# zerenluo123/legged_gym

Measured on AMD Instinct MI355X. Metric: env-steps/sec (whole node), Go1 rough-terrain 4096 envs/GPU at 1/2/4/8 GPUs, higher is better.
Workload: dtype fp32; 1 GPU; C3 go1_rough: Go1 trimesh curriculum terrain + 187-point height scan, actuator-net history+MLP, PPO 24 steps x 4096 envs/GPU, 5 epochs x 4 minibatches; envs_per_gpu=4096, global_envs=4096, parallelism=dp1

## Files before the change

legged_gym_amd/csrc/lgx_api.hip:

```cpp
#include <stdio.h>
#include <string.h>

#include <new>
#include <string>
#include <vector>

#include "lgx_internal.h"

static thread_local std::string g_err;

static int fail(int code, const char* msg) {
  g_err = msg;
  return code;
}
static int hip_check(hipError_t e, const char* what) {
  if (e == hipSuccess) return 0;
  char buf[256];
  snprintf(buf, sizeof buf, "%s: %s", what, hipGetErrorString(e));
  g_err = buf;
  return LGX_EHIP;
}
int lgx_fail(int code, const char* msg) { return fail(code, msg); }
int lgx_hip_status(const char* what) { return hip_check(hipGetLastError(), what); }
static int launch_check(int rc, const char* what) {
  if (rc == 0) return 0;
  if (rc == -1) return fail(LGX_EINVAL, what);
  return hip_check(hipGetLastError(), what);
}

struct lgx_sim {
  int device;
  bool dense;
  int pp;
  int act_mode;
  int32_t num_points;
  lgx_env_params params;
  lgx_buffers bufs;
  lgx_dev_model* d_model;
  lgx_env_params* d_params;
  const float* draws;
  float* extras_snapshot;
  lgx_priv_args priv;
  lgx_hist_args hist;
  lgx_act_rand_args arand;
  hipStream_t aux;
  hipEvent_t aux_in, aux_done;
  bool aux_pending;
  int32_t n_term_rows;
  int32_t profiling;
  int64_t prof_calls;
  std::vector<hipEvent_t> ev[3];
  std::vector<hipEvent_t> pool;
};

static hipEvent_t take_event(lgx_sim* s) {
  if (!s->pool.empty()) { hipEvent_t e = s->pool.back(); s->pool.pop_back(); return e; }
  hipEvent_t e = nullptr;
  if (hipEventCreateWithFlags(&e, hipEventDisableSystemFence) != hipSuccess) return nullptr;
  return e;
}
thread_local lgx_timing_slot lgx_timing;

static void arm(lgx_sim* s, int cls, bool sample) {
  lgx_timing = lgx_timing_slot{};
  if (!sample) return;
  hipEvent_t e0 = take_event(s), e1 = take_event(s);
// ... 80 lines not shown
  lgx_dev_model dm;
  memset(&dm, 0, sizeof dm);
  dm.m = *model;
  dm.m.leg_dof = leg_dof;
  int rr = 0;
  for (int i = 0; i < (dense ? 0 : model->num_points); ++i) {
    int d = model->point_dyn[i];
    int rep = model->point_report[i];
    if (d < 0 || d >= LGX_NUM_DYN) return fail(LGX_EINVAL, "lgx_sim_create: bad point_dyn");
    int lane;
    if (d == 0) {
      if (rep != 0) return fail(LGX_EINVAL, "lgx_sim_create: base points must report on body 0");
      lane = rr++ & 3;
    } else {
      lane = (d - 1) / 3;
      if (rep < 1 + 4 * lane || rep > 4 + 4 * lane) return fail(LGX_EINVAL, "lgx_sim_create: leg point reports on a foreign body");
    }
    if (dm.lane_npts[lane] >= LGX_MAX_LANE_PTS) return fail(LGX_EINVAL, "lgx_sim_create: too many contact points per leg");
    dm.lane_pts[lane][dm.lane_npts[lane]++] = i;
  }
  for (int l = 0; l < 4; ++l) dm.max_lane_npts = dm.lane_npts[l] > dm.max_lane_npts ? dm.lane_npts[l] : dm.max_lane_npts;
  dm.joint_rot_eye = 1;
  for (int j = 0; j < LGX_NUM_DOF; ++j)
    for (int i = 0; i < 9; ++i)
      if (model->joint_rot[j][i] != (i % 4 == 0 ? 1.f : 0.f)) dm.joint_rot_eye = 0;

  int rc = hip_check(hipSetDevice(device), "hipSetDevice");
  if (rc) return rc;
  lgx_sim* s = new (std::nothrow) lgx_sim();
  if (!s) return fail(LGX_ENOMEM, "lgx_sim_create: out of host memory");
  s->device = device;
  s->dense = dense;
  s->pp = lgx_physics_pp(params->num_envs);
  const char* am = getenv("LGX_ACT_OVERLAP");
  s->act_mode = am && *am ? atoi(am) : 2;
  if (s->act_mode < 0 || s->act_mode > 2 || (am && *am && (am[0] < '0' || am[0] > '2' || am[1]))) {
    delete s;
    return fail(LGX_EINVAL, "lgx_sim_create: LGX_ACT_OVERLAP must be 0, 1 or 2");
  }
  s->num_points = model->num_points;
  s->params = *params;
  s->bufs = *bufs;
  s->draws = nullptr;
  s->extras_snapshot = nullptr;
  s->priv = lgx_priv_args{};
  s->hist = lgx_hist_args{};
  s->arand = lgx_act_rand_args{};
  s->aux = nullptr;
  s->aux_in = s->aux_done = nullptr;
  s->aux_pending = false;
  s->profiling = 0;
  s->prof_calls = 0;
  s->n_term_rows = params->num_terms + (params->termination_slot >= 0 ? 1 : 0);
  if ((rc = hip_check(hipMalloc(&s->d_model, sizeof(lgx_dev_model)), "hipMalloc(model)"))) { delete s; return rc; }
  if ((rc = hip_check(hipMalloc(&s->d_params, sizeof(lgx_env_params)), "hipMalloc(params)"))) {
    (void)hipFree(s->d_model); delete s; return rc;
  }
  rc = hip_check(hipMemcpy(s->d_model, &dm, sizeof dm, hipMemcpyHostToDevice), "hipMemcpy(model)");
  if (!rc) rc = hip_check(hipMemcpy(s->d_params, params, sizeof *params, hipMemcpyHostToDevice), "hipMemcpy(params)");
  if (!rc) {
    const int64_t blocks = (params->num_envs + LGX_ENV_BLOCK - 1) / LGX_ENV_BLOCK;
    rc = hip_check(hipMemset(bufs->scratch + blocks * LGX_PARTIAL_STRIDE, 0, sizeof(unsigned int)), "hipMemset(ticket)");
  }
  if (rc) { (void)hipFree(s->d_model); (void)hipFree(s->d_params); delete s; return rc; }
  *out = s;
  return 0;
// ... 179 lines not shown
  if (ctrl == LGX_CTRL_T && (d->kp_scale || d->kd_scale))
    return fail(LGX_EINVAL, "lgx_bind_actuator_rand: LGX_CTRL_T has no gains to scale");
  const size_t bytes = sizeof(float) * (size_t)s->params.num_envs * LGX_NUM_DOF;
  float* prev = s->arand.prev;
  if (!prev) {
    if (int rc = hip_check(hipMalloc(&prev, bytes), "lgx_bind_actuator_rand: hipMalloc(prev)")) return rc;
  }
  s->arand = lgx_act_rand_args{d->kp_scale, d->kd_scale, d->lag, prev};
  if (int rc = hip_check(hipDeviceSynchronize(), "lgx_bind_actuator_rand: hipDeviceSynchronize")) return rc;
  if (int rc = hip_check(hipMemset(prev, 0, bytes), "lgx_bind_actuator_rand: hipMemset(prev)")) return rc;
  return hip_check(hipDeviceSynchronize(), "lgx_bind_actuator_rand: hipDeviceSynchronize");
}

int lgx_rebind_extras(lgx_sim* s, float* snapshot) {
  if (!s) return fail(LGX_EINVAL, "lgx_rebind_extras: null sim");
  s->extras_snapshot = snapshot;
  return 0;
}

static int join_aux(lgx_sim* s, hipStream_t st) {
  if (!s->aux_pending) return 0;
  return hip_check(hipStreamWaitEvent(st, s->aux_done, 0), "hipStreamWaitEvent(aux)");
}


int lgx_sync_aux(lgx_sim* s, void* stream) {
  if (!s) return fail(LGX_EINVAL, "lgx_sync_aux: null sim");
  return join_aux(s, (hipStream_t)stream);
}

static int physics(lgx_sim* s, int32_t nsub, int32_t from_actions, const float* actions, hipStream_t st, int32_t frozen) {
  if (s->arand.prev)
    return lgx_launch_physics_rand(s->d_model, s->d_params, s->bufs, s->params.num_envs, nsub, from_actions, actions,
                                   st, frozen, s->pp, s->arand);
  return s->dense ? lgx_launch_physics_dense(s->d_model, s->d_params, s->bufs, s->params.num_envs, nsub, from_actions,
                                             actions, st, frozen, s->num_points)
                  : lgx_launch_physics(s->d_model, s->d_params, s->bufs, s->params.num_envs, nsub, from_actions, actions,
                                       st, frozen, s->pp);
}

int lgx_simulate(lgx_sim* s, int32_t n, void* stream) {
  if (!s || n < 0) return fail(LGX_EINVAL, "lgx_simulate: bad arguments");
  if (n == 0) return 0;
  if (int rc = join_aux(s, (hipStream_t)stream)) return rc;
  return launch_check(physics(s, n, 0, nullptr, (hipStream_t)stream, 0), "lgx_simulate: physics launch");
}

int lgx_drive_inputs(lgx_sim* s, const float* actions, void* stream) {
  if (!s) return fail(LGX_EINVAL, "lgx_drive_inputs: null sim");
  if (int rc = join_aux(s, (hipStream_t)stream)) return rc;
  return launch_check(physics(s, s->params.decimation, 1, actions, (hipStream_t)stream, 1), "lgx_drive_inputs: launch");
}

int lgx_ground_contact(lgx_sim* s, const float* points, int32_t n, float* out, void* stream) {
  if (!s || n < 0 || (n > 0 && (!points || !out))) return fail(LGX_EINVAL, "lgx_ground_contact: bad arguments");
  return launch_check(lgx_launch_ground_contact(s->d_params, s->bufs, points, n, out, (hipStream_t)stream),
                      "lgx_ground_contact: launch");
}

int lgx_post_physics(lgx_sim* s, int64_t step, void* stream) {
  if (!s) return fail(LGX_EINVAL, "lgx_post_physics: null sim");
  return launch_check(lgx_launch_post_physics(s->d_params, s->bufs, s->params.num_envs, s->params.num_obs, s->n_term_rows,
                                              s->params.measure_heights, step, s->draws, s->extras_snapshot, s->priv,
                                              s->hist, (hipStream_t)stream),
                      "lgx_post_physics: launch");
}

static int post_physics_fused(lgx_sim* s, int64_t step, hipStream_t st, bool sample);

int lgx_step(lgx_sim* s, int64_t step, void* stream) { return lgx_step_from(s, nullptr, step, stream); }

// ... 200 lines not shown
```

legged_gym_amd/csrc/lgx_device.h:

```cpp
#pragma once
#include <hip/hip_runtime.h>
#include <stdint.h>

#include "../../include/lgx.h"

#define LGX_DEV __device__ __forceinline__

#ifdef LGX_PHASE_CLOCK
#include <stdio.h>
#define LGX_CLK_DECL(n) LGX_CLK_START uint64_t lgx_clk_acc[n] = {}; uint64_t lgx_clk_t = clock64();
#define LGX_CLK(i) do { const uint64_t _t = clock64(); lgx_clk_acc[i] += _t - lgx_clk_t; lgx_clk_t = _t; } while (0)
#ifdef LGX_PHASE_CLOCK_ALL
#define LGX_CLK_WHO (threadIdx.x == 0)
#else
#define LGX_CLK_WHO (blockIdx.x == 0 && threadIdx.x == 0)
#endif
#ifdef LGX_PHASE_CLOCK_BUF
#define LGX_CLK_MAXB 4096
static __device__ unsigned long long lgx_clk_buf[LGX_CLK_MAXB][14];
#define LGX_CLK_START const unsigned long long lgx_clk_t0 = __builtin_amdgcn_s_memrealtime();
#define LGX_CLK_PRINT(name, n)                                                                        \
  if (threadIdx.x == 0 && blockIdx.x < LGX_CLK_MAXB) {                                                \
    lgx_clk_buf[blockIdx.x][0] = lgx_clk_t0;                                                          \
    lgx_clk_buf[blockIdx.x][1] = __builtin_amdgcn_s_memrealtime();                                    \
    for (int _i = 0; _i < n && _i < 12; ++_i) lgx_clk_buf[blockIdx.x][2 + _i] = lgx_clk_acc[_i];      \
  }
#else
#define LGX_CLK_START
#define LGX_CLK_PRINT(name, n)                                                                        \
  if (LGX_CLK_WHO) {      \
    unsigned long long _v[12] = {};                                                                   \
    for (int _i = 0; _i < n && _i < 12; ++_i) _v[_i] = lgx_clk_acc[_i];                               \
    printf("%s cycles: b=%d 0=%llu 1=%llu 2=%llu 3=%llu 4=%llu 5=%llu 6=%llu 7=%llu 8=%llu 9=%llu "   \
           "10=%llu 11=%llu\n", name, (int)blockIdx.x, _v[0], _v[1], _v[2], _v[3], _v[4], _v[5], _v[6],  \
           _v[7], _v[8], _v[9], _v[10], _v[11]);                                                       \
  }
#endif
#else
#define LGX_CLK_DECL(n)
#define LGX_CLK(i) do { } while (0)
#define LGX_CLK_PRINT(name, n)
#endif

LGX_DEV void lgx_uniform4(uint64_t seed, int32_t env, int32_t slot4, int64_t step, uint32_t tag, float out[4]) {
  uint32_t c0 = (uint32_t)env, c1 = (uint32_t)slot4, c2 = (uint32_t)step;
  uint32_t c3 = tag ^ ((uint32_t)((uint64_t)step >> 32) << 8);
  uint32_t k0 = (uint32_t)seed, k1 = (uint32_t)(seed >> 32);
#pragma unroll
  for (int r = 0; r < 10; ++r) {
    uint32_t lo0 = 0xD2511F53u * c0, hi0 = __umulhi(0xD2511F53u, c0);
    uint32_t lo1 = 0xCD9E8D57u * c2, hi1 = __umulhi(0xCD9E8D57u, c2);
    uint32_t n0 = hi1 ^ c1 ^ k0, n2 = hi0 ^ c3 ^ k1;
    c0 = n0; c1 = lo1; c2 = n2; c3 = lo0;
    k0 += 0x9E3779B9u; k1 += 0xBB67AE85u;
  }
  const float s = 1.0f / 16777216.0f;
  out[0] = (float)(c0 >> 8) * s; out[1] = (float)(c1 >> 8) * s;
  out[2] = (float)(c2 >> 8) * s; out[3] = (float)(c3 >> 8) * s;
// ... 127 lines not shown
```

legged_gym_amd/csrc/lgx_internal.h:

```cpp
#pragma once
#include <hip/hip_ext.h>
#include <hip/hip_runtime.h>

#include "../../include/lgx.h"

#define LGX_MAX_LANE_PTS 24

struct lgx_dev_model {
  lgx_model m;
  int32_t lane_npts[4];
  int32_t max_lane_npts;
  int32_t joint_rot_eye;
  int32_t lane_pts[4][LGX_MAX_LANE_PTS];
  int32_t pad_tail[(4 - (sizeof(lgx_model) / 4 + 6 + 4 * LGX_MAX_LANE_PTS) % 4) % 4];
};

int lgx_launch_ground_contact(const lgx_env_params* dp, const lgx_buffers& b, const float* q, int32_t n, float* o,
                              hipStream_t stream);
int lgx_physics_pp(int32_t n_envs);
int lgx_launch_physics(const lgx_dev_model* dm, const lgx_env_params* dp, const lgx_buffers& b, int32_t n_envs,
                       int32_t nsub, int32_t from_actions, const float* act_src, hipStream_t stream, int32_t frozen,
                       int pp);
struct lgx_act_rand_args {
  const float* kp_scale;
  const float* kd_scale;
  const int32_t* lag;
  float* prev;
};
int lgx_launch_physics_rand(const lgx_dev_model* dm, const lgx_env_params* dp, const lgx_buffers& b, int32_t n_envs,
                            int32_t nsub, int32_t from_actions, const float* act_src, hipStream_t stream,
                            int32_t frozen, int pp, const lgx_act_rand_args& ar);
int lgx_launch_physics_dense(const lgx_dev_model* dm, const lgx_env_params* dp, const lgx_buffers& b, int32_t n_envs,
                             int32_t nsub, int32_t from_actions, const float* act_src, hipStream_t stream,
                             int32_t frozen, int32_t num_points);
struct lgx_priv_args {
  float* buf;
  int32_t width, num_terms;
  uint32_t ids;
  uint32_t pad;
  uint64_t offs_lo, offs_hi;
  float cf_scale, tq_scale;
  __host__ __device__ int id(int t) const { return (int)((ids >> (4 * t)) & 15u); }
  __host__ __device__ int off(int t) const { return (int)(((t < 4 ? offs_lo : offs_hi) >> (16 * (t & 3))) & 0xffffu); }
  void set(int t, int id_, int off_) {
    ids |= (uint32_t)id_ << (4 * t);
    (t < 4 ? offs_lo : offs_hi) |= (uint64_t)off_ << (16 * (t & 3));
  }
};
static_assert(LGX_PRIV_MAX_TERMS <= 8 && LGX_PRIV_COUNT <= 16 && LGX_MAX_PRIV_OBS < 65536, "lgx_priv_args packing");
struct lgx_hist_args {
  float* row;
  const float* prev;
  int32_t* age;
  int32_t frames, frame_width, width;
};
int lgx_launch_post_physics(const lgx_env_params* dp, const lgx_buffers& b, int32_t n_envs, int32_t num_obs,
                            int32_t n_term_rows, int32_t measure_heights, int64_t step, const float* draws,
                            float* extras_snapshot, const lgx_priv_args& pv, const lgx_hist_args& hv,
                            hipStream_t stream);
int lgx_launch_post_physics_act(const lgx_env_params* dp, const lgx_buffers& b, int32_t n_envs, int64_t step,
                                const float* draws, float* extras_snapshot, const float* act_in, float* act_out,
                                int64_t act_rows, const float* act_w, const float* act_scale,
                                const lgx_priv_args& pv, const lgx_hist_args& hv, hipStream_t stream);
int lgx_launch_post_physics_hist(const lgx_env_params* dp, const lgx_buffers& b, int32_t n_envs, int64_t step,
// ... 84 lines not shown
```

legged_gym_amd/csrc/lgx_physics.hip:

```cpp
#include <stdlib.h>

#include "lgx_device.h"
#include "lgx_internal.h"

namespace {

struct sv { f3 a, l; };
LGX_DEV sv sv0() { return sv{mk3(0, 0, 0), mk3(0, 0, 0)}; }
LGX_DEV sv add(sv x, sv y) { return sv{x.a + y.a, x.l + y.l}; }
LGX_DEV sv scale(float s, sv x) { return sv{s * x.a, s * x.l}; }
LGX_DEV float dot(sv x, sv y) { return dot(x.a, y.a) + dot(x.l, y.l); }
LGX_DEV sv crm(sv V, sv s) { return sv{cross(V.a, s.a), cross(V.a, s.l) + cross(V.l, s.a)}; }
LGX_DEV sv crf(sv V, sv f) { return sv{cross(V.a, f.a) + cross(V.l, f.l), cross(V.a, f.l)}; }

struct SI { float m; f3 h; float I[6]; };
LGX_DEV SI si_add(const SI& x, const SI& y) {
  SI r; r.m = x.m + y.m; r.h = x.h + y.h;
#pragma unroll
  for (int i = 0; i < 6; ++i) r.I[i] = x.I[i] + y.I[i];
  return r;
}
LGX_DEV sv si_mul(const SI& s, sv v) {
  f3 Ia = mk3(s.I[0] * v.a.x + s.I[3] * v.a.y + s.I[4] * v.a.z, s.I[3] * v.a.x + s.I[1] * v.a.y + s.I[5] * v.a.z,
              s.I[4] * v.a.x + s.I[5] * v.a.y + s.I[2] * v.a.z);
  return sv{Ia + cross(s.h, v.l), cross(v.a, s.h) + s.m * v.l};
}
LGX_DEV SI body_si(const lgx_model* __restrict__ M, int b, float scale, const m33& R, f3 o) {
  const float* in = M->body_inertia[b];
  m33 Ib = {{in[0], in[3], in[4], in[3], in[1], in[5], in[4], in[5], in[2]}};
  m33 T = mul(R, Ib);
  float Iw[6];
  Iw[0] = T.a[0] * R.a[0] + T.a[1] * R.a[1] + T.a[2] * R.a[2];
  Iw[1] = T.a[3] * R.a[3] + T.a[4] * R.a[4] + T.a[5] * R.a[5];
// ... 514 lines not shown
}

LGX_DEV void wave_lds_sync() {
  __builtin_amdgcn_fence(__ATOMIC_RELEASE, "wavefront");
  __builtin_amdgcn_wave_barrier();
  __builtin_amdgcn_fence(__ATOMIC_ACQUIRE, "wavefront");
}

}

#define MAX_LANE_PTS LGX_MAX_LANE_PTS
#ifndef LGX_PHYS_WAVES_PER_SIMD
#define LGX_PHYS_WAVES_PER_SIMD 1
#endif
#define HIST_STRIDE 31

template <int PP>
LGX_DEV float psum(float v) {
  if (PP == 4) return row_quads_sum(v);
  if (PP >= 2) v += lane_xor4(v);
  if (PP >= 4) v += lane_xor8(v);
  if (PP >= 8) v += __shfl_xor(v, 16);
  return v;
}

#define PHYS_KP(k, j) (RAND ? arow[k] : M->kp[j])
#define PHYS_KD(k, j) (RAND ? arow[3 + (k)] : M->kd[j])
#define PHYS_PG(k, j) (RAND ? arow[k] : P->p_gains[j])
#define PHYS_DG(k, j) (RAND ? arow[3 + (k)] : P->d_gains[j])
#define PHYS_AE(k) (RAND ? ae_lag[k] : act[k])
LGX_DEV lgx_act_rand_args act_rand_of() { return lgx_act_rand_args{nullptr, nullptr, nullptr, nullptr}; }
LGX_DEV lgx_act_rand_args act_rand_of(const lgx_act_rand_args& a) { return a; }

template <int PP, typename... AR>
__global__ void __launch_bounds__(64 * PP, LGX_PHYS_WAVES_PER_SIMD)
lgx_physics_kernel(const lgx_dev_model* __restrict__ DMg, const lgx_env_params* __restrict__ P, lgx_buffers B,
                   int32_t nsub, int32_t from_actions, const float* __restrict__ act_src, int32_t frozen, AR... ar) {
  static_assert(sizeof...(AR) <= 1, "at most the actuator tables");
  constexpr bool RAND = sizeof...(AR) == 1;
  constexpr int PHYS_BLOCK = 64 * PP;
  constexpr int LPE = 4 * PP;
  constexpr int SLOTS = (MAX_LANE_PTS + PP - 1) / PP;
  constexpr int ENVS = 16;
  __shared__ lgx_dev_model smodel;
  __shared__ float4 slot_state[SLOTS][PHYS_BLOCK];
  __shared__ float4 geo_p[SLOTS][PHYS_BLOCK];
  __shared__ float4 geo_n[SLOTS][PHYS_BLOCK];
  __shared__ float hist_lds[ENVS * 4 * HIST_STRIDE];
  __shared__ float leg_kin[ENVS * 4][3][12];
  __shared__ float leg_sys[ENVS * 4][36];
  __shared__ float env_com[ENVS][40];
  __shared__ int32_t hf_patch[ENVS][LGX_HF_PATCH * LGX_HF_PATCH];
  __shared__ int32_t hf_org[ENVS][2];
  __shared__ uint32_t tm_q[PP][64 * SLOTS];
  {
    static_assert(sizeof(lgx_dev_model) % 16 == 0, "the model is staged in 16-byte units");
    const int4* src = reinterpret_cast<const int4*>(DMg);
    int4* dst = reinterpret_cast<int4*>(&smodel);
    for (int i = threadIdx.x; i < (int)(sizeof(lgx_dev_model) / 16); i += PHYS_BLOCK) dst[i] = src[i];
    __syncthreads();
  }
  const lgx_dev_model* DM = &smodel;
  const lgx_model* M = &smodel.m;
  const int tid = threadIdx.x;
  const int gl = blockIdx.x * PHYS_BLOCK + tid;
  const int e = gl / LPE;
  const int lie = gl % LPE;
  const int eb = tid / LPE;
  const int leg = lie & 3;
  const int pl = lie >> 2;
// ... 340 lines not shown
      for (int sl = 0; sl < SLOTS; ++sl) {
        if (sl >= nslots) break;
        const bool act = pl + PP * sl < npts;
        const int pi = slot_pt[sl];
        const int db = slot_db[sl];
        const int k = db == 0 ? -1 : (db - 1) % 3;
        const float* fr = db == 0 ? ecom + 27 : kin + 12 * k;
        m33 R;
#pragma unroll
        for (int i = 0; i < 9; ++i) R.a[i] = fr[i];
        f3 ol = db == 0 ? mk3(0, 0, 0) : mk3(fr[9], fr[10], fr[11]);
        f3 Pp = ol + mul(R, mk3(M->point_pos[pi][0], M->point_pos[pi][1], M->point_pos[pi][2]));
        const float rad = M->point_radius[pi];
        f3 n;
        bool defer;
        const float depth = ground_cell(P, B, Pp + pos, rad, &n, patch, pi0, pj0, &defer);
        defer = defer && act;
        const uint64_t m = __ballot(defer);
        if (defer) {
          tm_q[wv][qn + __popcll(m & below)] = (uint32_t)(sl << 6 | ln);
          geo_p[sl][tid] = make_float4(Pp.x, Pp.y, Pp.z, rad);
          geo_n[sl][tid] = make_float4(0.f, 0.f, 1.f, (float)pi);
        } else if (act) {
          slot_state[sl][tid] = make_float4(depth > 0.f ? 1.f : 0.f, 0.f, 0.f, 0.f);
          if (depth > 0.f) {
            const f3 Pc = Pp - rad * n;
            geo_p[sl][tid] = make_float4(Pc.x, Pc.y, Pc.z, depth);
            geo_n[sl][tid] = make_float4(n.x, n.y, n.z, (float)pi);
          }
        }
        qn += __popcll(m);
      }
      LGX_CLK(8);
      if (qn > 0) {
        wave_lds_sync();
        const bool cull1 = qn > 16;
        int qn2 = 0;
        for (int q0 = 0; q0 < qn; q0 += 64) {
          const int q = q0 + ln;
          uint32_t ent = 0;
          unsigned keep = 0;
          if (q < qn) {
            ent = tm_q[wv][q];
            const int sl2 = (ent >> 6) & 1023, t = (wv << 6) | (ent & 63), e2 = t / LPE;
            const float4 g = geo_p[sl2][t];
            const f3 pw = mk3(g.x, g.y, g.z) + mk3(env_com[e2][36], env_com[e2][37], env_com[e2][38]);
            const int32_t* hp = use_patch ? hf_patch[e2] : nullptr;
            const int o0 = use_patch ? hf_org[e2][0] : 0, o1 = use_patch ? hf_org[e2][1] : 0;
            int i, j;
            tm_cell(P, B, pw, &i, &j);
            if (cull1) {
              f3 pl3;
              keep = tm_keep(P, B, pw, g.w, i, j, hp, o0, o1, &pl3);
            } else {
              keep = tm_near(P, B, pw, g.w, i, j, hp, o0, o1) ? 0x1ffu : 0u;
            }
            if (!keep) slot_state[sl2][t] = make_float4(0.f, 0.f, 0.f, 0.f);
          }
          const uint64_t m = __ballot(keep != 0);
          if (keep) tm_q[wv][qn2 + __popcll(m & below)] = ent | keep << 16;
          qn2 += __popcll(m);
        }
        wave_lds_sync();
        LGX_CLK(9);
#ifdef LGX_PHASE_CLOCK
        lgx_clk_acc[11] += (uint64_t)qn * 1000 + qn2;
#endif
        if (qn2 <= 8) {
          const int grp = ln >> 4, g = ln & 15;
          for (int q0 = 0; q0 < qn2; q0 += 4) {
            const int q = min(q0 + grp, qn2 - 1);
            const uint32_t ent = tm_q[wv][q];
            const int sl2 = (ent >> 6) & 1023, t = (wv << 6) | (ent & 63), e2 = t / LPE;
            const float4 gp = geo_p[sl2][t];
            const f3 Pp = mk3(gp.x, gp.y, gp.z);
            const f3 pw = Pp + mk3(env_com[e2][36], env_com[e2][37], env_com[e2][38]);
            const int32_t* hp = use_patch ? hf_patch[e2] : nullptr;
            const int o0 = use_patch ? hf_org[e2][0] : 0, o1 = use_patch ? hf_org[e2][1] : 0;
            int i, j;
            tm_cell(P, B, pw, &i, &j);
            const f3 pl3 = tm_local(P, pw, i, j);
            TmQuery tq;
            tm_init(tq, pl3);
            if (g < 9 && ((ent >> (16 + g)) & 1u))
              tm_cell_tris(tq, P, B, pl3, gp.w, i, j, (g * 11) >> 5, g - 3 * ((g * 11) >> 5), hp, o0, o1);
            int cd2 = g, ctop = g;
            tm_combine_step<1>(tq, cd2, ctop);
            tm_combine_step<2>(tq, cd2, ctop);
            tm_combine_step<4>(tq, cd2, ctop);
            tm_combine_step<8>(tq, cd2, ctop);
            if (g == 0 && q0 + grp < qn2) {
              f3 n;
              const float depth = tm_finish(tq, pl3, gp.w, &n);
              slot_state[sl2][t] = make_float4(depth > 0.f ? 1.f : 0.f, 0.f, 0.f, 0.f);
              if (depth > 0.f) {
                const f3 Pc = Pp - gp.w * n;
                geo_p[sl2][t] = make_float4(Pc.x, Pc.y, Pc.z, depth);
                geo_n[sl2][t] = make_float4(n.x, n.y, n.z, geo_n[sl2][t].w);
              }
            }
          }
        } else {
          for (int q0 = 0; q0 < qn2; q0 += 64) {
            const int q = q0 + ln;
            if (q < qn2) {
              const uint32_t ent = tm_q[wv][q];
              const int sl2 = (ent >> 6) & 1023, t = (wv << 6) | (ent & 63), e2 = t / LPE;
              const float4 gp = geo_p[sl2][t];
              const f3 Pp = mk3(gp.x, gp.y, gp.z);
              const f3 pw = Pp + mk3(env_com[e2][36], env_com[e2][37], env_com[e2][38]);
              int i, j;
              tm_cell(P, B, pw, &i, &j);
              f3 n;
              const float depth = tm_visit(P, B, tm_local(P, pw, i, j), gp.w, i, j, ent >> 16, &n,
                                           use_patch ? hf_patch[e2] : nullptr, use_patch ? hf_org[e2][0] : 0,
                                           use_patch ? hf_org[e2][1] : 0);
              slot_state[sl2][t] = make_float4(depth > 0.f ? 1.f : 0.f, 0.f, 0.f, 0.f);
              if (depth > 0.f) {
                const f3 Pc = Pp - gp.w * n;
                geo_p[sl2][t] = make_float4(Pc.x, Pc.y, Pc.z, depth);
                geo_n[sl2][t] = make_float4(n.x, n.y, n.z, geo_n[sl2][t].w);
              }
            }
          }
        }
      }
      wave_lds_sync();
    }
    uint32_t own_act = 0;
    {
      float sx[SLOTS];
#pragma unroll
      for (int sl = 0; sl < SLOTS; ++sl) sx[sl] = slot_state[sl][tid].x;
#pragma unroll
      for (int sl = 0; sl < SLOTS; ++sl)
        own_act |= ((unsigned)(pl + PP * sl < npts) & (unsigned)(sx[sl] != 0.f)) << sl;
    }
    LGX_CLK(10);
    float xb[6];
    f3 xl;
    for (int pass = 0; pass < 2; ++pass) {
      LegSys L;
#pragma unroll
      for (int i = 0; i < 21; ++i) L.Ap[i] = 0.f;
#pragma unroll
      for (int i = 0; i < 6; ++i) { L.rb[i] = 0.f; L.B[i][0] = L.B[i][1] = L.B[i][2] = 0.f; }
#pragma unroll
      for (int i = 0; i < 6; ++i) L.D[i] = 0.f;
      L.rl[0] = L.rl[1] = L.rl[2] = 0.f;
      uint32_t w = own_act;
#pragma unroll 1
      for (int trip = 0; trip < SLOTS; ++trip) {
        if (__ballot(w != 0u) == 0) break;
        const bool on = w != 0u;
        const int sl = on ? __builtin_ctz(w) : 0;
        w &= w - 1;
        const float4 st = slot_state[sl][tid];
// ... 153 lines not shown
    float* to = B.dof_targets + (int64_t)e * 12 + leg * 3;
    to[0] = tgt[0]; to[1] = tgt[1]; to[2] = tgt[2];
  }
  float* cfo = B.contact_forces + (int64_t)e * LGX_MAX_BODIES * 3;
#pragma unroll
  for (int r = 0; r < 4; ++r) {
    float* d = cfo + (1 + 4 * leg + r) * 3;
    d[0] = cf_leg[r].x; d[1] = cf_leg[r].y; d[2] = cf_leg[r].z;
  }
  if (use_hist) {
    float* h = B.act_hist + (int64_t)e * 120 + leg * 30;
#pragma unroll
    for (int i = 0; i < 30; i += 2) *reinterpret_cast<float2*>(h + i) = make_float2(hist[i], hist[i + 1]);
  }
  if (lane0) {
    cfo[0] = cf_base.x; cfo[1] = cf_base.y; cfo[2] = cf_base.z;
    float* ro = B.root_states + (int64_t)e * 13;
    ro[0] = pos.x; ro[1] = pos.y; ro[2] = pos.z;
    ro[3] = qx; ro[4] = qy; ro[5] = qz; ro[6] = qw;
    ro[7] = vlin.x; ro[8] = vlin.y; ro[9] = vlin.z;
    ro[10] = wang.x; ro[11] = wang.y; ro[12] = wang.z;
  }
  LGX_CLK(7);
  LGX_CLK_PRINT("physics", 12)
#if defined(LGX_PHASE_CLOCK) && !defined(LGX_PHASE_CLOCK_BUF)
  if (LGX_CLK_WHO)
    printf("physics bodies: b=%d pass0=%u pass1=%u classify=%u report=%u\n", (int)blockIdx.x, lgx_bodies[0],
           lgx_bodies[1], lgx_bodies[2], lgx_bodies[3]);
#elif defined(LGX_PHASE_CLOCK)
  (void)lgx_bodies;
#endif
}

#ifdef LGX_PHYSICS_RAND

int lgx_launch_physics_rand(const lgx_dev_model* dm, const lgx_env_params* dp, const lgx_buffers& b, int32_t n_envs,
                            int32_t nsub, int32_t from_actions, const float* act_src, hipStream_t stream,
                            int32_t frozen, int ppx, const lgx_act_rand_args& ar) {
  if (!ar.prev) return -1;
  if (!act_src) act_src = b.actions;
  const int blocks = (n_envs + 15) / 16;
  if (ppx == 8)
    LGX_LAUNCH((lgx_physics_kernel<8, lgx_act_rand_args>), dim3(blocks), dim3(512), 0, stream, dm, dp, b, nsub,
               from_actions, act_src, frozen, ar);
  else if (ppx == 4)
    LGX_LAUNCH((lgx_physics_kernel<4, lgx_act_rand_args>), dim3(blocks), dim3(256), 0, stream, dm, dp, b, nsub,
               from_actions, act_src, frozen, ar);
  else if (ppx == 2)
    LGX_LAUNCH((lgx_physics_kernel<2, lgx_act_rand_args>), dim3(blocks), dim3(128), 0, stream, dm, dp, b, nsub,
               from_actions, act_src, frozen, ar);
  else
    LGX_LAUNCH((lgx_physics_kernel<1, lgx_act_rand_args>), dim3(blocks), dim3(64), 0, stream, dm, dp, b, nsub,
               from_actions, act_src, frozen, ar);
  return hipGetLastError() == hipSuccess ? 0 : -2;
}

#else

__global__ void lgx_ground_contact_kernel(const lgx_env_params* __restrict__ P, lgx_buffers B, const float4* __restrict__ q,
                                          int32_t n, float4* __restrict__ o) {
  const int k = blockIdx.x * blockDim.x + threadIdx.x;
  if (k >= n) return;
  const float4 v = q[k];
  f3 nn;
  const float d = ground_contact(P, B, mk3(v.x, v.y, v.z), v.w, &nn, nullptr, 0, 0);
  o[k] = make_float4(d, nn.x, nn.y, nn.z);
}

int lgx_launch_ground_contact(const lgx_env_params* dp, const lgx_buffers& b, const float* q, int32_t n, float* o,
                              hipStream_t stream) {
  if (n <= 0) return 0;
  hipLaunchKernelGGL(lgx_ground_contact_kernel, dim3((n + 255) / 256), dim3(256), 0, stream, dp, b,
                     reinterpret_cast<const float4*>(q), n, reinterpret_cast<float4*>(o));
  return hipGetLastError() == hipSuccess ? 0 : -2;
}

int lgx_physics_pp(int32_t n_envs) {
  (void)n_envs;
  const char* force = getenv("LGX_PHYS_PP");
  const int f = force ? atoi(force) : 0;
  return (f == 1 || f == 2 || f == 4 || f == 8) ? f : 4;
}

int lgx_launch_physics(const lgx_dev_model* dm, const lgx_env_params* dp, const lgx_buffers& b, int32_t n_envs,
                       int32_t nsub, int32_t from_actions, const float* act_src, hipStream_t stream, int32_t frozen,
                       int ppx) {
  if (!act_src) act_src = b.actions;
  const int blocks = (n_envs + 15) / 16;
  if (ppx == 8)
    LGX_LAUNCH(lgx_physics_kernel<8>, dim3(blocks), dim3(512), 0, stream, dm, dp, b, nsub, from_actions, act_src, frozen);
  else if (ppx == 4)
    LGX_LAUNCH(lgx_physics_kernel<4>, dim3(blocks), dim3(256), 0, stream, dm, dp, b, nsub, from_actions, act_src, frozen);
  else if (ppx == 2)
    LGX_LAUNCH(lgx_physics_kernel<2>, dim3(blocks), dim3(128), 0, stream, dm, dp, b, nsub, from_actions, act_src, frozen);
  else
    LGX_LAUNCH(lgx_physics_kernel<1>, dim3(blocks), dim3(64), 0, stream, dm, dp, b, nsub, from_actions, act_src, frozen);
  return hipGetLastError() == hipSuccess ? 0 : -2;
}


namespace {

constexpr int DN = 18;
constexpr int DCF = 3 * DN + 3 + 3 + 1 + 1 + 3 + 3;

struct DenseLds {
  float R[LGX_NUM_DYN][9], o[LGX_NUM_DYN][3], S[LGX_NUM_DOF][6], I6[LGX_NUM_DYN][36];
  float H[DN * DN], M[DN * DN];
  float V[LGX_NUM_DYN][6], A[LGX_NUM_DYN][6], F[LGX_NUM_DYN][6];
  float ICroot[4][36], Froot[4][6];
  float Cb[DN], g[DN], Hu[DN], r[DN], u[DN], u2[DN];
  float th[12], thd[12], tgt[12], tex[12], Dimp[12];
  float root[13];
  int impl[12];
  int nc;
};

struct DenseContacts {
  float (*J)[3 * DN];
  float (*P)[3];
  float (*n)[3];
  float* depth;
  float* mu;
  float (*fs)[3];
  float (*f)[3];
  int* body;
  int* report;
  int* stat;
};
// ... 479 lines not shown
      const f3 q = mk3(L.root[3], L.root[4], L.root[5]);
      const float qw = L.root[6];
      const f3 wq = cross(w, q);
      float dq[4] = {0.5f * (qw * w.x + wq.x), 0.5f * (qw * w.y + wq.y), 0.5f * (qw * w.z + wq.z), -0.5f * dot(w, q)};
      float qq[4] = {q.x + dt * dq[0], q.y + dt * dq[1], q.z + dt * dq[2], qw + dt * dq[3]};
      const float qn = 1.0f / sqrtf(qq[0] * qq[0] + qq[1] * qq[1] + qq[2] * qq[2] + qq[3] * qq[3]);
      L.root[3] = qq[0] * qn; L.root[4] = qq[1] * qn; L.root[5] = qq[2] * qn; L.root[6] = qq[3] * qn;
      L.root[7] = v.x; L.root[8] = v.y; L.root[9] = v.z;
      L.root[10] = w.x; L.root[11] = w.y; L.root[12] = w.z;
    }
    __syncthreads();
  }
  if (lane < 12) {
    B.dof_state[(int64_t)e * 24 + 2 * lane] = L.th[lane];
    B.dof_state[(int64_t)e * 24 + 2 * lane + 1] = L.thd[lane];
    if (ctrl != LGX_CTRL_POS_DRIVE && nsub > 0) B.torques[(int64_t)e * 12 + lane] = L.tex[lane];
  }
  if (lane < 13) B.root_states[(int64_t)e * 13 + lane] = L.root[lane];
}

static int lgx_physics_dense_lds(int32_t num_points) { return num_points * (DCF + 3) * 4; }

int lgx_launch_physics_dense(const lgx_dev_model* dm, const lgx_env_params* dp, const lgx_buffers& b, int32_t n_envs,
                             int32_t nsub, int32_t from_actions, const float* act_src, hipStream_t stream,
                             int32_t frozen, int32_t num_points) {
  if (!act_src) act_src = b.actions;
  const int cap = num_points > 0 ? num_points : 1;
  LGX_LAUNCH(lgx_physics_dense_kernel, dim3(n_envs), dim3(64), lgx_physics_dense_lds(cap), stream, dm, dp, b, nsub,
             from_actions, act_src, frozen, cap);
  return hipGetLastError() == hipSuccess ? 0 : -2;
}

#ifdef LGX_PHASE_CLOCK_BUF
extern "C" int lgx_debug_clock(unsigned long long* out, int32_t nblocks) {
  return hipMemcpyFromSymbol(out, HIP_SYMBOL(lgx_clk_buf), (size_t)min(nblocks, LGX_CLK_MAXB) * 14 * 8, 0,
                             hipMemcpyDeviceToHost) == hipSuccess ? 0 : -1;
}
#endif

#endif
```

Measured before the change: 6.079 million env-steps/s.

## Add workgroup-pooled 16-lane trimesh query mode with auto selection

Splits the narrow-phase trimesh contact stage into a lambda-based stage-1 cull and a reusable 16-lanes-per-query round routine. It adds a new kernel variant that pools the queued queries of all waves in a workgroup through LDS counts and __syncthreads, so they are spread evenly across the whole block. An LGX_PHYS_TMQ env knob picks the mode. The auto mode picks the pooled kernel when the model has more than 32 sphere points, and otherwise uses the 16-lane form whenever the first-stage cull was skipped. The aim is to fix load imbalance and the poor lane use of one-query-per-lane processing. In exchange it adds block barriers and another kernel instantiation, and the debug clock buffer becomes per-wave.

```diff
diff --git a/legged_gym_amd/csrc/lgx_api.hip b/legged_gym_amd/csrc/lgx_api.hip
--- a/legged_gym_amd/csrc/lgx_api.hip
+++ b/legged_gym_amd/csrc/lgx_api.hip
@@ -32,6 +32,7 @@
   int device;
   bool dense;
   int pp;
+  int tmq;
   int act_mode;
   int32_t num_points;
   lgx_env_params params;
@@ -178,6 +179,16 @@
   s->device = device;
   s->dense = dense;
   s->pp = lgx_physics_pp(params->num_envs);
+  s->tmq = lgx_physics_tmq();
+  if (s->tmq < 0) {
+    delete s;
+    return fail(LGX_EINVAL, "lgx_sim_create: LGX_PHYS_TMQ must be auto, parent, wave16, wave1 or wg16");
+  }
+  if (s->tmq == LGX_TMQ_AUTO) {
+    int spheres = 0;
+    for (int i = 0; i < model->num_points; ++i) spheres += model->point_radius[i] > 0.f;
+    if (spheres > 32) s->tmq = LGX_TMQ_WG16;
+  }
   const char* am = getenv("LGX_ACT_OVERLAP");
   s->act_mode = am && *am ? atoi(am) : 2;
   if (s->act_mode < 0 || s->act_mode > 2 || (am && *am && (am[0] < '0' || am[0] > '2' || am[1]))) {
@@ -423,11 +434,11 @@
 static int physics(lgx_sim* s, int32_t nsub, int32_t from_actions, const float* actions, hipStream_t st, int32_t frozen) {
   if (s->arand.prev)
     return lgx_launch_physics_rand(s->d_model, s->d_params, s->bufs, s->params.num_envs, nsub, from_actions, actions,
-                                   st, frozen, s->pp, s->arand);
+                                   st, frozen, s->pp, s->tmq, s->arand);
   return s->dense ? lgx_launch_physics_dense(s->d_model, s->d_params, s->bufs, s->params.num_envs, nsub, from_actions,
                                              actions, st, frozen, s->num_points)
                   : lgx_launch_physics(s->d_model, s->d_params, s->bufs, s->params.num_envs, nsub, from_actions, actions,
-                                       st, frozen, s->pp);
+                                       st, frozen, s->pp, s->tmq);
 }
 
 int lgx_simulate(lgx_sim* s, int32_t n, void* stream) {
diff --git a/legged_gym_amd/csrc/lgx_device.h b/legged_gym_amd/csrc/lgx_device.h
--- a/legged_gym_amd/csrc/lgx_device.h
+++ b/legged_gym_amd/csrc/lgx_device.h
@@ -16,14 +16,20 @@
 #define LGX_CLK_WHO (blockIdx.x == 0 && threadIdx.x == 0)
 #endif
 #ifdef LGX_PHASE_CLOCK_BUF
-#define LGX_CLK_MAXB 4096
-static __device__ unsigned long long lgx_clk_buf[LGX_CLK_MAXB][14];
-#define LGX_CLK_START const unsigned long long lgx_clk_t0 = __builtin_amdgcn_s_memrealtime();
+#define LGX_CLK_MAXW 8192
+#define LGX_CLK_COLS 18
+static __device__ unsigned long long lgx_clk_buf[LGX_CLK_MAXW][LGX_CLK_COLS];
+#define LGX_CLK_START const unsigned long long lgx_clk_t0 = __builtin_amdgcn_s_memrealtime(); \
+  unsigned long long lgx_clk_q[4] = {0ull, 0ull, 0ull, 0ull};
 #define LGX_CLK_PRINT(name, n)                                                                        \
-  if (threadIdx.x == 0 && blockIdx.x < LGX_CLK_MAXB) {                                                \
-    lgx_clk_buf[blockIdx.x][0] = lgx_clk_t0;                                                          \
-    lgx_clk_buf[blockIdx.x][1] = __builtin_amdgcn_s_memrealtime();                                    \
-    for (int _i = 0; _i < n && _i < 12; ++_i) lgx_clk_buf[blockIdx.x][2 + _i] = lgx_clk_acc[_i];      \
+  {                                                                                                   \
+    const unsigned _w = blockIdx.x * (blockDim.x >> 6) + (threadIdx.x >> 6);                          \
+    if ((threadIdx.x & 63) == 0 && _w < LGX_CLK_MAXW) {                                               \
+      lgx_clk_buf[_w][0] = lgx_clk_t0;                                                                \
+      lgx_clk_buf[_w][1] = __builtin_amdgcn_s_memrealtime();                                          \
+      for (int _i = 0; _i < n && _i < 12; ++_i) lgx_clk_buf[_w][2 + _i] = lgx_clk_acc[_i];            \
+      for (int _i = 0; _i < 4; ++_i) lgx_clk_buf[_w][14 + _i] = lgx_clk_q[_i];                        \
+    }                                                                                                 \
   }
 #else
 #define LGX_CLK_START
diff --git a/legged_gym_amd/csrc/lgx_internal.h b/legged_gym_amd/csrc/lgx_internal.h
--- a/legged_gym_amd/csrc/lgx_internal.h
+++ b/legged_gym_amd/csrc/lgx_internal.h
@@ -18,9 +18,17 @@
 int lgx_launch_ground_contact(const lgx_env_params* dp, const lgx_buffers& b, const float* q, int32_t n, float* o,
                               hipStream_t stream);
 int lgx_physics_pp(int32_t n_envs);
+enum {
+  LGX_TMQ_AUTO = 0,
+  LGX_TMQ_PARENT = 1,
+  LGX_TMQ_WAVE16 = 2,
+  LGX_TMQ_WAVE1 = 3,
+  LGX_TMQ_WG16 = 4,
+};
+int lgx_physics_tmq(void);
 int lgx_launch_physics(const lgx_dev_model* dm, const lgx_env_params* dp, const lgx_buffers& b, int32_t n_envs,
                        int32_t nsub, int32_t from_actions, const float* act_src, hipStream_t stream, int32_t frozen,
-                       int pp);
+                       int pp, int tmq);
 struct lgx_act_rand_args {
   const float* kp_scale;
   const float* kd_scale;
@@ -29,7 +37,7 @@
 };
 int lgx_launch_physics_rand(const lgx_dev_model* dm, const lgx_env_params* dp, const lgx_buffers& b, int32_t n_envs,
                             int32_t nsub, int32_t from_actions, const float* act_src, hipStream_t stream,
-                            int32_t frozen, int pp, const lgx_act_rand_args& ar);
+                            int32_t frozen, int pp, int tmq, const lgx_act_rand_args& ar);
 int lgx_launch_physics_dense(const lgx_dev_model* dm, const lgx_env_params* dp, const lgx_buffers& b, int32_t n_envs,
                              int32_t nsub, int32_t from_actions, const float* act_src, hipStream_t stream,
                              int32_t frozen, int32_t num_points);
diff --git a/legged_gym_amd/csrc/lgx_physics.hip b/legged_gym_amd/csrc/lgx_physics.hip
--- a/legged_gym_amd/csrc/lgx_physics.hip
+++ b/legged_gym_amd/csrc/lgx_physics.hip
@@ -1,4 +1,5 @@
 #include <stdlib.h>
+#include <string.h>
 
 #include "lgx_device.h"
 #include "lgx_internal.h"
@@ -579,10 +580,10 @@
 LGX_DEV lgx_act_rand_args act_rand_of() { return lgx_act_rand_args{nullptr, nullptr, nullptr, nullptr}; }
 LGX_DEV lgx_act_rand_args act_rand_of(const lgx_act_rand_args& a) { return a; }
 
-template <int PP, typename... AR>
-__global__ void __launch_bounds__(64 * PP, LGX_PHYS_WAVES_PER_SIMD)
-lgx_physics_kernel(const lgx_dev_model* __restrict__ DMg, const lgx_env_params* __restrict__ P, lgx_buffers B,
-                   int32_t nsub, int32_t from_actions, const float* __restrict__ act_src, int32_t frozen, AR... ar) {
+template <int PP, bool WG, typename... AR>
+LGX_DEV void lgx_physics_body(const lgx_dev_model* __restrict__ DMg, const lgx_env_params* __restrict__ P,
+                              lgx_buffers B, int32_t nsub, int32_t from_actions,
+                              const float* __restrict__ act_src, int32_t frozen, int32_t tmq, AR... ar) {
   static_assert(sizeof...(AR) <= 1, "at most the actuator tables");
   constexpr bool RAND = sizeof...(AR) == 1;
   constexpr int PHYS_BLOCK = 64 * PP;
@@ -989,9 +990,7 @@
         qn += __popcll(m);
       }
       LGX_CLK(8);
-      if (qn > 0) {
-        wave_lds_sync();
-        const bool cull1 = qn > 16;
+      auto stage1 = [&](const bool cull1) {
         int qn2 = 0;
         for (int q0 = 0; q0 < qn; q0 += 64) {
           const int q = q0 + ln;
@@ -1018,68 +1017,117 @@
           if (keep) tm_q[wv][qn2 + __popcll(m & below)] = ent | keep << 16;
           qn2 += __popcll(m);
         }
-        wave_lds_sync();
-        LGX_CLK(9);
-#ifdef LGX_PHASE_CLOCK
-        lgx_clk_acc[11] += (uint64_t)qn * 1000 + qn2;
+        return qn2;
+      };
+      auto rounds16 = [&](const int tot, const int grp, const int rows, auto entry_of) {
+        const int g = ln & 15;
+        for (int q0 = 0; q0 < tot; q0 += rows) {
+          int w2;
+          const int q = entry_of(min(q0 + grp, tot - 1), w2);
+          const uint32_t ent = tm_q[w2][q];
+          const int sl2 = (ent >> 6) & 1023, t = (w2 << 6) | (ent & 63), e2 = t / LPE;
+          const float4 gp = geo_p[sl2][t];
+          const f3 Pp = mk3(gp.x, gp.y, gp.z);
+          const f3 pw = Pp + mk3(env_com[e2][36], env_com[e2][37], env_com[e2][38]);
+          const int32_t* hp = use_patch ? hf_patch[e2] : nullptr;
+          const int o0 = use_patch ? hf_org[e2][0] : 0, o1 = use_patch ? hf_org[e2][1] : 0;
+          int i, j;
+          tm_cell(P, B, pw, &i, &j);
+          const f3 pl3 = tm_local(P, pw, i, j);
+          TmQuery tq;
+          tm_init(tq, pl3);
+          if (g < 9 && ((ent >> (16 + g)) & 1u))
+            tm_cell_tris(tq, P, B, pl3, gp.w, i, j, (g * 11) >> 5, g - 3 * ((g * 11) >> 5), hp, o0, o1);
+          int cd2 = g, ctop = g;
+          tm_combine_step<1>(tq, cd2, ctop);
+          tm_combine_step<2>(tq, cd2, ctop);
+          tm_combine_step<4>(tq, cd2, ctop);
+          tm_combine_step<8>(tq, cd2, ctop);
+          if (g == 0 && q0 + grp < tot) {
+            f3 n;
+            const float depth = tm_finish(tq, pl3, gp.w, &n);
+            slot_state[sl2][t] = make_float4(depth > 0.f ? 1.f : 0.f, 0.f, 0.f, 0.f);
+            if (depth > 0.f) {
+              const f3 Pc = Pp - gp.w * n;
+              geo_p[sl2][t] = make_float4(Pc.x, Pc.y, Pc.z, depth);
+              geo_n[sl2][t] = make_float4(n.x, n.y, n.z, geo_n[sl2][t].w);
+            }
+          }
+        }
+      };
+      if constexpr (!WG) {
+        if (qn > 0) {
+          wave_lds_sync();
+          const bool cull1 = tmq == LGX_TMQ_WAVE1 || qn > 16;
+          const int qn2 = stage1(cull1);
+          wave_lds_sync();
+          LGX_CLK(9);
+          const bool form16 = tmq == LGX_TMQ_WAVE16 ||
+                              (tmq != LGX_TMQ_WAVE1 && (qn2 <= 8 || (tmq == LGX_TMQ_AUTO && !cull1)));
+#ifdef LGX_PHASE_CLOCK_BUF
+          if (s < 4) lgx_clk_q[s] = (unsigned long long)qn << 32 | (unsigned long long)qn2 << 16 | (form16 ? 1u : 0u);
 #endif
-        if (qn2 <= 8) {
-          const int grp = ln >> 4, g = ln & 15;
-          for (int q0 = 0; q0 < qn2; q0 += 4) {
-            const int q = min(q0 + grp, qn2 - 1);
-            const uint32_t ent = tm_q[wv][q];
-            const int sl2 = (ent >> 6) & 1023, t = (wv << 6) | (ent & 63), e2 = t / LPE;
-            const float4 gp = geo_p[sl2][t];
-            const f3 Pp = mk3(gp.x, gp.y, gp.z);
-            const f3 pw = Pp + mk3(env_com[e2][36], env_com[e2][37], env_com[e2][38]);
-            const int32_t* hp = use_patch ? hf_patch[e2] : nullptr;
-            const int o0 = use_patch ? hf_org[e2][0] : 0, o1 = use_patch ? hf_org[e2][1] : 0;
-            int i, j;
-            tm_cell(P, B, pw, &i, &j);
-            const f3 pl3 = tm_local(P, pw, i, j);
-            TmQuery tq;
-            tm_init(tq, pl3);
-            if (g < 9 && ((ent >> (16 + g)) & 1u))
-              tm_cell_tris(tq, P, B, pl3, gp.w, i, j, (g * 11) >> 5, g - 3 * ((g * 11) >> 5), hp, o0, o1);
-            int cd2 = g, ctop = g;
-            tm_combine_step<1>(tq, cd2, ctop);
-            tm_combine_step<2>(tq, cd2, ctop);
-            tm_combine_step<4>(tq, cd2, ctop);
-            tm_combine_step<8>(tq, cd2, ctop);
-            if (g == 0 && q0 + grp < qn2) {
-              f3 n;
-              const float depth = tm_finish(tq, pl3, gp.w, &n);
-              slot_state[sl2][t] = make_float4(depth > 0.f ? 1.f : 0.f, 0.f, 0.f, 0.f);
-              if (depth > 0.f) {
-                const f3 Pc = Pp - gp.w * n;
-                geo_p[sl2][t] = make_float4(Pc.x, Pc.y, Pc.z, depth);
-                geo_n[sl2][t] = make_float4(n.x, n.y, n.z, geo_n[sl2][t].w);
+          if (form16) {
+            rounds16(qn2, ln >> 4, 4, [&](int q, int& w2) { w2 = wv; return q; });
+          } else {
+            for (int q0 = 0; q0 < qn2; q0 += 64) {
+              const int q = q0 + ln;
+#ifdef LGX_PHASE_CLOCK_BUF
+              {
+                int mc = q < qn2 ? __popc(tm_q[wv][q] >> 16) : 0;
+                for (int o = 32; o; o >>= 1) mc = max(mc, __shfl_xor(mc, o));
+                if (s < 4 && (unsigned long long)mc > ((lgx_clk_q[s] >> 8) & 255))
+                  lgx_clk_q[s] = (lgx_clk_q[s] & ~0xff00ull) | (unsigned long long)mc << 8;
+              }
+#endif
+              if (q < qn2) {
+                const uint32_t ent = tm_q[wv][q];
+                const int sl2 = (ent >> 6) & 1023, t = (wv << 6) | (ent & 63), e2 = t / LPE;
+                const float4 gp = geo_p[sl2][t];
+                const f3 Pp = mk3(gp.x, gp.y, gp.z);
+                const f3 pw = Pp + mk3(env_com[e2][36], env_com[e2][37], env_com[e2][38]);
+                int i, j;
+                tm_cell(P, B, pw, &i, &j);
+                f3 n;
+                const float depth = tm_visit(P, B, tm_local(P, pw, i, j), gp.w, i, j, ent >> 16, &n,
+                                             use_patch ? hf_patch[e2] : nullptr, use_patch ? hf_org[e2][0] : 0,
+                                             use_patch ? hf_org[e2][1] : 0);
+                slot_state[sl2][t] = make_float4(depth > 0.f ? 1.f : 0.f, 0.f, 0.f, 0.f);
+                if (depth > 0.f) {
+                  const f3 Pc = Pp - gp.w * n;
+                  geo_p[sl2][t] = make_float4(Pc.x, Pc.y, Pc.z, depth);
+                  geo_n[sl2][t] = make_float4(n.x, n.y, n.z, geo_n[sl2][t].w);
+                }
               }
             }
           }
-        } else {
-          for (int q0 = 0; q0 < qn2; q0 += 64) {
-            const int q = q0 + ln;
-            if (q < qn2) {
-              const uint32_t ent = tm_q[wv][q];
-              const int sl2 = (ent >> 6) & 1023, t = (wv << 6) | (ent & 63), e2 = t / LPE;
-              const float4 gp = geo_p[sl2][t];
-              const f3 Pp = mk3(gp.x, gp.y, gp.z);
-              const f3 pw = Pp + mk3(env_com[e2][36], env_com[e2][37], env_com[e2][38]);
-              int i, j;
-              tm_cell(P, B, pw, &i, &j);
-              f3 n;
-              const float depth = tm_visit(P, B, tm_local(P, pw, i, j), gp.w, i, j, ent >> 16, &n,
-                                           use_patch ? hf_patch[e2] : nullptr, use_patch ? hf_org[e2][0] : 0,
-                                           use_patch ? hf_org[e2][1] : 0);
-              slot_state[sl2][t] = make_float4(depth > 0.f ? 1.f : 0.f, 0.f, 0.f, 0.f);
-              if (depth > 0.f) {
-                const f3 Pc = Pp - gp.w * n;
-                geo_p[sl2][t] = make_float4(Pc.x, Pc.y, Pc.z, depth);
-                geo_n[sl2][t] = make_float4(n.x, n.y, n.z, geo_n[sl2][t].w);
-              }
-            }
-          }
+        }
+      } else {
+        __shared__ int32_t tm_cnt[PP];
+        const bool tm_launch = P->terrain_kind != 0 && B.hf_trimesh != nullptr;
+        int qn2 = 0;
+        if (qn > 0) {
+          wave_lds_sync();
+          qn2 = stage1(qn > 16);
+        }
+        LGX_CLK(9);
+        if (tm_launch) {
+          if (ln == 0) tm_cnt[wv] = qn2;
+          __syncthreads();
+          int cnt[PP], tot = 0;
+#pragma unroll
+          for (int w = 0; w < PP; ++w) { cnt[w] = tm_cnt[w]; tot += cnt[w]; }
+#ifdef LGX_PHASE_CLOCK_BUF
+          if (s < 4) lgx_clk_q[s] = (unsigned long long)qn << 32 | (unsigned long long)qn2 << 16 | 1u;
+#endif
+          rounds16(tot, tid >> 4, 4 * PP, [&](int q, int& w2) {
+            w2 = 0;
+#pragma unroll
+            for (int w = 0; w < PP - 1; ++w)
+              if (w2 == w && q >= cnt[w]) { q -= cnt[w]; w2 = w + 1; }
+            return q;
+          });
+          __syncthreads();
         }
       }
       wave_lds_sync();
@@ -1299,26 +1347,45 @@
 #endif
 }
 
+template <int PP, typename... AR>
+__global__ void __launch_bounds__(64 * PP, LGX_PHYS_WAVES_PER_SIMD)
+lgx_physics_kernel(const lgx_dev_model* __restrict__ DMg, const lgx_env_params* __restrict__ P, lgx_buffers B,
+                   int32_t nsub, int32_t from_actions, const float* __restrict__ act_src, int32_t frozen, int32_t tmq,
+                   AR... ar) {
+  lgx_physics_body<PP, false, AR...>(DMg, P, B, nsub, from_actions, act_src, frozen, tmq, ar...);
+}
+
+template <int PP, typename... AR>
+__global__ void __launch_bounds__(64 * PP, LGX_PHYS_WAVES_PER_SIMD)
+lgx_physics_wg_kernel(const lgx_dev_model* __restrict__ DMg, const lgx_env_params* __restrict__ P, lgx_buffers B,
+                      int32_t nsub, int32_t from_actions, const float* __restrict__ act_src, int32_t frozen,
+                      int32_t tmq, AR... ar) {
+  lgx_physics_body<PP, true, AR...>(DMg, P, B, nsub, from_actions, act_src, frozen, tmq, ar...);
+}
+
 #ifdef LGX_PHYSICS_RAND
 
 int lgx_launch_physics_rand(const lgx_dev_model* dm, const lgx_env_params* dp, const lgx_buffers& b, int32_t n_envs,
                             int32_t nsub, int32_t from_actions, const float* act_src, hipStream_t stream,
-                            int32_t frozen, int ppx, const lgx_act_rand_args& ar) {
+                            int32_t frozen, int ppx, int tmq, const lgx_act_rand_args& ar) {
   if (!ar.prev) return -1;
   if (!act_src) act_src = b.actions;
   const int blocks = (n_envs + 15) / 16;
-  if (ppx == 8)
-    LGX_LAUNCH((lgx_physics_kernel<8, lgx_act_rand_args>), dim3(blocks), dim3(512), 0, stream, dm, dp, b, nsub,
-               from_actions, act_src, frozen, ar);
-  else if (ppx == 4)
-    LGX_LAUNCH((lgx_physics_kernel<4, lgx_act_rand_args>), dim3(blocks), dim3(256), 0, stream, dm, dp, b, nsub,
-               from_actions, act_src, frozen, ar);
-  else if (ppx == 2)
-    LGX_LAUNCH((lgx_physics_kernel<2, lgx_act_rand_args>), dim3(blocks), dim3(128), 0, stream, dm, dp, b, nsub,
-               from_actions, act_src, frozen, ar);
-  else
-    LGX_LAUNCH((lgx_physics_kernel<1, lgx_act_rand_args>), dim3(blocks), dim3(64), 0, stream, dm, dp, b, nsub,
-               from_actions, act_src, frozen, ar);
+#define PHYS_RAND_LAUNCH(K)                                                                                     \
+  if (ppx == 8)                                                                                                  \
+    LGX_LAUNCH((K<8, lgx_act_rand_args>), dim3(blocks), dim3(512), 0, stream, dm, dp, b, nsub, from_actions,     \
+               act_src, frozen, tmq, ar);                                                                        \
+  else if (ppx == 4)                                                                                             \
+    LGX_LAUNCH((K<4, lgx_act_rand_args>), dim3(blocks), dim3(256), 0, stream, dm, dp, b, nsub, from_actions,     \
+               act_src, frozen, tmq, ar);                                                                        \
+  else if (ppx == 2)                                                                                             \
+    LGX_LAUNCH((K<2, lgx_act_rand_args>), dim3(blocks), dim3(128), 0, stream, dm, dp, b, nsub, from_actions,     \
+               act_src, frozen, tmq, ar);                                                                        \
+  else                                                                                                           \
+    LGX_LAUNCH((K<1, lgx_act_rand_args>), dim3(blocks), dim3(64), 0, stream, dm, dp, b, nsub, from_actions,      \
+               act_src, frozen, tmq, ar);
+  if (tmq == LGX_TMQ_WG16) { PHYS_RAND_LAUNCH(lgx_physics_wg_kernel) } else { PHYS_RAND_LAUNCH(lgx_physics_kernel) }
+#undef PHYS_RAND_LAUNCH
   return hipGetLastError() == hipSuccess ? 0 : -2;
 }
 
@@ -1349,19 +1416,32 @@
   return (f == 1 || f == 2 || f == 4 || f == 8) ? f : 4;
 }
 
+int lgx_physics_tmq(void) {
+  const char* v = getenv("LGX_PHYS_TMQ");
+  if (!v || !*v || !strcmp(v, "auto")) return LGX_TMQ_AUTO;
+  if (!strcmp(v, "parent")) return LGX_TMQ_PARENT;
+  if (!strcmp(v, "wave16")) return LGX_TMQ_WAVE16;
+  if (!strcmp(v, "wave1")) return LGX_TMQ_WAVE1;
+  if (!strcmp(v, "wg16")) return LGX_TMQ_WG16;
+  return -1;
+}
+
 int lgx_launch_physics(const lgx_dev_model* dm, const lgx_env_params* dp, const lgx_buffers& b, int32_t n_envs,
                        int32_t nsub, int32_t from_actions, const float* act_src, hipStream_t stream, int32_t frozen,
-                       int ppx) {
+                       int ppx, int tmq) {
   if (!act_src) act_src = b.actions;
   const int blocks = (n_envs + 15) / 16;
-  if (ppx == 8)
-    LGX_LAUNCH(lgx_physics_kernel<8>, dim3(blocks), dim3(512), 0, stream, dm, dp, b, nsub, from_actions, act_src, frozen);
-  else if (ppx == 4)
-    LGX_LAUNCH(lgx_physics_kernel<4>, dim3(blocks), dim3(256), 0, stream, dm, dp, b, nsub, from_actions, act_src, frozen);
-  else if (ppx == 2)
-    LGX_LAUNCH(lgx_physics_kernel<2>, dim3(blocks), dim3(128), 0, stream, dm, dp, b, nsub, from_actions, act_src, frozen);
-  else
-    LGX_LAUNCH(lgx_physics_kernel<1>, dim3(blocks), dim3(64), 0, stream, dm, dp, b, nsub, from_actions, act_src, frozen);
+#define PHYS_LAUNCH(K)                                                                                           \
+  if (ppx == 8)                                                                                                  \
+    LGX_LAUNCH(K<8>, dim3(blocks), dim3(512), 0, stream, dm, dp, b, nsub, from_actions, act_src, frozen, tmq);   \
+  else if (ppx == 4)                                                                                             \
+    LGX_LAUNCH(K<4>, dim3(blocks), dim3(256), 0, stream, dm, dp, b, nsub, from_actions, act_src, frozen, tmq);   \
+  else if (ppx == 2)                                                                                             \
+    LGX_LAUNCH(K<2>, dim3(blocks), dim3(128), 0, stream, dm, dp, b, nsub, from_actions, act_src, frozen, tmq);   \
+  else                                                                                                           \
+    LGX_LAUNCH(K<1>, dim3(blocks), dim3(64), 0, stream, dm, dp, b, nsub, from_actions, act_src, frozen, tmq);
+  if (tmq == LGX_TMQ_WG16) { PHYS_LAUNCH(lgx_physics_wg_kernel) } else { PHYS_LAUNCH(lgx_physics_kernel) }
+#undef PHYS_LAUNCH
   return hipGetLastError() == hipSuccess ? 0 : -2;
 }
 
@@ -1907,8 +1987,8 @@
 }
 
 #ifdef LGX_PHASE_CLOCK_BUF
-extern "C" int lgx_debug_clock(unsigned long long* out, int32_t nblocks) {
-  return hipMemcpyFromSymbol(out, HIP_SYMBOL(lgx_clk_buf), (size_t)min(nblocks, LGX_CLK_MAXB) * 14 * 8, 0,
+extern "C" int lgx_debug_clock(unsigned long long* out, int32_t nwaves) {
+  return hipMemcpyFromSymbol(out, HIP_SYMBOL(lgx_clk_buf), (size_t)min(nwaves, LGX_CLK_MAXW) * LGX_CLK_COLS * 8, 0,
                              hipMemcpyDeviceToHost) == hipSuccess ? 0 : -1;
 }
 #endif
```

Result: no change. 6.112 million env-steps/s, median of 2 (+0.5%).
